# SFXiang/ORB-SLAM2-Annotation

Measured on AMD Instinct MI355X. Metric: frames/sec ORB extract+match (1000 feat, 640×480 mono) at 1/2/4/8 GPU; % HBM roofline, higher is better.
Workload: dtype u8

## Files before the change

### include/orbgpu_debug.h

```cpp
#ifndef ORBGPU_DEBUG_H
#define ORBGPU_DEBUG_H

#include "orbgpu.h"

#ifdef __cplusplus
extern "C" {
#endif

int orbgpu_debug_level_candidates(orbgpu_extractor* ex, int frame, int level, int* xys, int cap);

int orbgpu_debug_level_octree(orbgpu_extractor* ex, int frame, int level, int* xys, int cap);

int orbgpu_debug_level_blur(orbgpu_extractor* ex, int frame, int level, uint8_t* dst, size_t dst_step);

int orbgpu_debug_octree_trace(orbgpu_extractor* ex, int enable, int* out, int cap);

int orbgpu_debug_pyramid_emulate(int nfeatures, float scale_factor, int nlevels, int width, int height,
                                 const uint8_t* img, size_t img_step, uint8_t* out, size_t out_bytes, int* info);

int orbgpu_debug_pyramid_plan_rows(int nfeatures, float scale_factor, int nlevels, int width, int height, int* rows,
                                   size_t rows_n, int* lane_info, size_t lanes_n, int* dims);

int orbgpu_debug_qr_solve_6x4_device(const double* A, const double* b, double* X, int n, void* stream);

#ifdef __cplusplus
}
#endif
#endif
```

### orb-slam2-annotation_amd/csrc/extractor.cpp

```cpp
#include <algorithm>
#include <atomic>
#include <chrono>
#include <cstring>
#include <memory>
#include <string>

#include "extractor.h"

using namespace orbgpu;

namespace {

int pyr_levels_max_batch() { return ORB_ENV_ONCE_INT("ORBGPU_PYR_LEVELS_MAX_BATCH", 8); }

int od_chunks() {
    const int n = env_now_int("ORBGPU_OD_CHUNKS", 1);
    return n < 1 ? 1 : (n > 8 ? 8 : n);
}

bool single_zero_copy() { return ORB_ENV_ONCE_FLAG("ORBGPU_SINGLE_ZEROCOPY", true); }

bool single_done_flag() { return ORB_ENV_ONCE_FLAG("ORBGPU_SINGLE_DONE_FLAG", true); }

bool single_vram_staging() { return ORB_ENV_ONCE_FLAG("ORBGPU_SINGLE_VRAM_STAGING", true); }

bool pyr_bands_off() { return !ORB_ENV_ONCE_FLAG("ORBGPU_PYR_BANDS", true); }

int run_batch(orbgpu_extractor* e, const uint8_t* imgs, int batch, size_t row_step, size_t frame_step,
              orbgpu_keypoint* kps, uint8_t* desc, int* counts, int kp_cap, hipStream_t s, int* err_copy = nullptr) {
    const Geom& g = e->geo.g;
    Event* evs = nullptr;
    if (e->profile) {
        if (e->ev_used == e->ev.size()) {
            std::array<Event, 5> a;
            for (Event& x : a) ORB_HIP(hipEventCreateWithFlags(x.put(), hipEventDisableSystemFence));
            e->ev.push_back(std::move(a));
        }
        evs = e->ev[e->ev_used++].data();
        ORB_HIP(hipEventRecord(evs[0], s));
    }
    if (batch <= pyr_levels_max_batch() && g.bd_nb > 0 && !pyr_bands_off())
        ORB_HIP(launch_pyramid_bands(g, batch, e->d_band, e->d_xtab, e->d_ytab, imgs, row_step, frame_step, e->d_pyr, s));
    else if (batch <= pyr_levels_max_batch())
        ORB_HIP(launch_pyramid_levels(g, batch, e->d_xtab, e->d_ytab, imgs, row_step, frame_step, e->d_pyr, s));
    else
        ORB_HIP(launch_pyramid(g, batch, e->d_pyr_ent, e->d_pyr_tab, imgs, row_step, frame_step, e->d_pyr, s));
    if (evs) ORB_HIP(hipEventRecord(evs[1], s));
    if (e->stage_ev[0]) ORB_HIP(hipEventRecord(e->stage_ev[0], s));
    ORB_HIP(launch_fast_cells(g, batch, imgs, row_step, frame_step, e->d_pyr, e->d_cand, e->d_cell_counts, e->d_err, s));
    if (evs) ORB_HIP(hipEventRecord(evs[2], s));
    if (e->stage_ev[1]) ORB_HIP(hipEventRecord(e->stage_ev[1], s));
    const int nch = (err_copy || batch < 16 * od_chunks()) ? 1 : od_chunks();
    if (nch == 1) {
        ORB_HIP(launch_octree(g, batch, e->d_cand, e->d_cell_counts, e->d_gkeys, e->d_gknode, e->d_oct_out,
                              e->d_oct_count, e->d_err, e->geo.oct_groups, 2, e->d_trace, s));
        if (evs) ORB_HIP(hipEventRecord(evs[3], s));
        if (e->stage_ev[2]) ORB_HIP(hipEventRecord(e->stage_ev[2], s));
        ORB_HIP(launch_describe(g, batch, imgs, row_step, frame_step, e->d_pyr, e->d_oct_out, e->d_oct_count, kps,
                                desc, counts, kp_cap, s, err_copy ? e->d_err.get() : nullptr, err_copy));
    } else {
        if (!e->aux_stream) {
            int lo = 0, hi = 0;
            ORB_HIP(hipDeviceGetStreamPriorityRange(&lo, &hi));
            ORB_HIP(hipStreamCreateWithPriority(e->aux_stream.put(), hipStreamNonBlocking, hi));
            for (Event& x : e->od_ev) ORB_HIP(hipEventCreateWithFlags(x.put(), hipEventDisableTiming));
        }
        hipStream_t a = e->aux_stream;
        for (int c = 0; c < nch; ++c) {
            const int f0 = batch * c / nch, f1 = batch * (c + 1) / nch, nb = f1 - f0;
            ORB_HIP(launch_octree(g, nb, e->d_cand + (size_t)f0 * g.cand_frame,
                                  e->d_cell_counts + (size_t)f0 * g.total_cells,
                                  e->d_gkeys + (size_t)f0 * g.cand_frame, e->d_gknode + (size_t)f0 * g.cand_frame,
                                  e->d_oct_out + (size_t)f0 * g.slots_frame, e->d_oct_count + (size_t)f0 * kOcStride,
                                  e->d_err, e->geo.oct_groups, 2, c == 0 ? e->d_trace.get() : nullptr, s));
            if (c == nch - 1 && evs) ORB_HIP(hipEventRecord(evs[3], s));
            ORB_HIP(hipEventRecord(e->od_ev[c], s));
            ORB_HIP(hipStreamWaitEvent(a, e->od_ev[c], 0));
            ORB_HIP(launch_describe(g, nb, imgs, row_step, frame_step, e->d_pyr, e->d_oct_out, e->d_oct_count, kps,
                                    desc, counts, kp_cap, a, nullptr, nullptr, f0));
        }
        if (e->stage_ev[2]) ORB_HIP(hipEventRecord(e->stage_ev[2], s));
        ORB_HIP(hipEventRecord(e->od_ev[8], a));
        ORB_HIP(hipStreamWaitEvent(s, e->od_ev[8], 0));
    }
    if (evs) ORB_HIP(hipEventRecord(evs[4], s));
    if (e->stage_ev[3]) ORB_HIP(hipEventRecord(e->stage_ev[3], s));
    e->last_img = imgs;
    e->last_row = row_step;
    e->last_frame = frame_step;
    e->last_batch = batch;
    return ORBGPU_OK;
}

std::string capacity_message(int err) {
    std::string m = "kernel capacity overflow:";
    if (err & kErrCellCap) m += " FAST-cell";
    if (err & kErrNodeCap) m += " octree-nodes";
    if (err & kErrKeyCap) m += " octree-keys";
    if (err & kErrSeqCap) m += " octree-seq";
    return m;
}

int collect_errors(orbgpu_extractor* e, hipStream_t s) {
    ORB_HIP(hipStreamSynchronize(s));
    int err = 0;
    ORB_HIP(hipMemcpy(&err, e->d_err, sizeof(int), hipMemcpyDeviceToHost));
    if (err) {
        ORB_HIP(hipMemset(e->d_err, 0, sizeof(int)));
        return fail(ORBGPU_ERR_CAPACITY, capacity_message(err));
    }
    return ORBGPU_OK;
}

template <class T>
hipError_t upload(T* dst, const std::vector<T>& src) {
    return src.empty() ? hipSuccess : hipMemcpy(dst, src.data(), src.size() * sizeof(T), hipMemcpyHostToDevice);
}

}

extern "C" {

int orbgpu_extractor_create(int nfeatures, float scale_factor, int nlevels, int ini_th, int min_th, int width,
                            int height, int max_batch, orbgpu_extractor** out) {
    if (!out) return fail(ORBGPU_ERR_ARG, "out is NULL");
    *out = nullptr;
    if (nfeatures <= 0 || nlevels <= 0 || nlevels > kMaxLevels || !(scale_factor > 1.f) || width <= 0 ||
// ... 352 lines not shown
```

### orb-slam2-annotation_amd/csrc/extractor_debug.cpp

```cpp
#include <algorithm>
#include <cstring>
#include <vector>

#include "../../include/orbgpu_debug.h"
#include "extractor.h"

using namespace orbgpu;

namespace {

int plan_geometry(int nfeatures, float scale_factor, int nlevels, int width, int height, ExtractorGeometry& geo,
                  GeometryTables& t) {
    return build_geometry(ExtractorParams{nfeatures, scale_factor, nlevels, 20, 7, width, height, 1}, geo, t);
}

}

extern "C" {

int orbgpu_debug_level_blur(orbgpu_extractor* e, int frame, int level, uint8_t* dst, size_t dst_step) {
    if (!e || !dst) return fail(ORBGPU_ERR_ARG, "NULL argument");
    DeviceScope ds_(e->device);
    if (!e->last_img || frame < 0 || frame >= e->last_batch || level < 0 || level >= e->p.nlevels)
        return fail(ORBGPU_ERR_ARG, "no such frame/level in the last extraction");
// ... 48 lines not shown
    if (out && e->d_trace) {
        ORB_HIP(hipDeviceSynchronize());
        ORB_HIP(hipMemcpy(out, e->d_trace, std::min(n, (size_t)cap) * sizeof(int), hipMemcpyDeviceToHost));
    }
    return ORBGPU_OK;
}

int orbgpu_debug_level_octree(orbgpu_extractor* e, int frame, int level, int* xys, int cap) {
    if (!e || frame < 0 || frame >= e->last_batch || level < 0 || level >= e->p.nlevels)
        return fail(ORBGPU_ERR_ARG, "no such frame/level in the last extraction");
    DeviceScope ds_(e->device);
    const Geom& g = e->geo.g;
    const LevelGeom& v = g.lv[level];
    int n = 0;
    ORB_HIP(hipDeviceSynchronize());
    ORB_HIP(hipMemcpy(&n, e->d_oct_count + (size_t)frame * kOcStride + level, sizeof(int), hipMemcpyDeviceToHost));
    std::vector<uint32_t> keys(std::max(n, 1));
    ORB_HIP(hipMemcpy(keys.data(), e->d_oct_out + (size_t)frame * g.slots_frame + v.out_offset,
                      (size_t)n * sizeof(uint32_t), hipMemcpyDeviceToHost));
    for (int i = 0; i < n && i < cap && xys; ++i) {
        xys[3 * i] = key_x(keys[i]); xys[3 * i + 1] = key_y(keys[i]); xys[3 * i + 2] = key_s(keys[i]);
    }
    return n;
}

int orbgpu_debug_pyramid_emulate(int nfeatures, float scale_factor, int nlevels, int width, int height,
                                 const uint8_t* img, size_t img_step, uint8_t* out, size_t out_bytes, int* info) {
    if (!img || !out || nfeatures <= 0 || nlevels <= 0 || nlevels > kMaxLevels || !(scale_factor > 1.f) ||
        width <= 0 || height <= 0 || img_step < (size_t)width)
        return fail(ORBGPU_ERR_ARG, "invalid emulation arguments");
    ExtractorGeometry geo;
    GeometryTables t;
    int rc = plan_geometry(nfeatures, scale_factor, nlevels, width, height, geo, t);
    if (rc) return rc;
    const Geom& g = geo.g;
    size_t need = 0;
    for (int l = 1; l < nlevels; ++l) need += (size_t)g.lv[l].w * g.lv[l].h;
    if (out_bytes < need) return fail(ORBGPU_ERR_CAPACITY, "out_bytes smaller than levels 1..L-1");
    std::vector<std::vector<uint8_t>> levels;
    rc = emulate_pyramid(g, t.ytab, geo.pyr_plan, img, img_step, levels);
    if (rc) return rc;
    for (int l = 1; l < nlevels; ++l) {
        std::memcpy(out, levels[(size_t)l].data(), levels[(size_t)l].size());
        out += levels[(size_t)l].size();
    }
    if (info) {
        const int v[8] = {g.tk_ticks, g.tk_t0, g.tk_cwaves, g.tk_pwaves, g.tk_np, g.tk_e, g.tk_lds_bytes,
                          g.lv[0].tk_ring_rows};
        std::memcpy(info, v, sizeof(v));
    }
    return ORBGPU_OK;
}

int orbgpu_debug_pyramid_plan_rows(int nfeatures, float scale_factor, int nlevels, int width, int height,
                                   int* rows, size_t rows_n, int* lane_info, size_t lanes_n, int* dims) {
    if (!dims || nfeatures <= 0 || nlevels < 2 || nlevels > kMaxLevels || !(scale_factor > 1.f) || width <= 0 ||
        height <= 0)
        return fail(ORBGPU_ERR_ARG, "invalid plan arguments");
    ExtractorGeometry geo;
    GeometryTables t;
    int rc = plan_geometry(nfeatures, scale_factor, nlevels, width, height, geo, t);
    if (rc) return rc;
    const Geom& g = geo.g;
    const int K = g.tk_ticks, CL = 64 * g.tk_cwaves, E = g.tk_e, n = CL * E;
    dims[0] = K;
    dims[1] = n;
    dims[2] = g.tk_cwaves;
    dims[3] = E;
    if (!rows || !lane_info) return ORBGPU_OK;
    if (rows_n < (size_t)K * n || lanes_n < (size_t)n) return fail(ORBGPU_ERR_CAPACITY, "plan output too small");
    const uint32_t* rng = reinterpret_cast<const uint32_t*>(geo.pyr_plan.tab.data()) + g.tk_rng;
    for (int i = 0; i < n; ++i) {
        const int4* r = &geo.pyr_plan.ent[(size_t)i * 9];
        lane_info[i] = r[2].w | (r[0].y ? 1 << 8 : 0);
        for (int k = 0; k < K; ++k) rows[(size_t)k * n + i] = (int)((rng[(size_t)k * g.tk_rs + r[0].x] >> 11) & 31u);
    }
    return ORBGPU_OK;
}

}
```

### orb-slam2-annotation_amd/csrc/octree.hip

```cpp
#include "orbgpu_internal.h"
#include "orbgpu_kernels.h"
#include "group_sum.h"
#include <algorithm>
#include <type_traits>

namespace orbgpu {

namespace {

#ifndef ORBGPU_OCT_THREADS
#define ORBGPU_OCT_THREADS 256
#endif
#ifndef ORBGPU_OCT_AGG_HIST
#define ORBGPU_OCT_AGG_HIST 1
#endif
constexpr bool kAggHist = ORBGPU_OCT_AGG_HIST != 0;
constexpr int kThreads = ORBGPU_OCT_THREADS;
#ifndef ORBGPU_OCT_THREADS_SMALL
#define ORBGPU_OCT_THREADS_SMALL 1024
#endif
constexpr int kThreadsSmall = ORBGPU_OCT_THREADS_SMALL;
constexpr int kSmallBatch = 8;

struct ONode {
// ... 169 lines not shown
        const int ex = incl - x;
        const unsigned long long br = __ballot(lane < m && nL + (ex - lane) + x - 1 >= N);
        const int kstop = br ? (int)__builtin_ctzll(br) : m - 1;
        C = kstop >= 0 ? __builtin_amdgcn_readlane(incl, kstop) : 0;
        if (lane == 0) s_misc[24] = kstop;
        if (lane < m) s_aux0[lane] = ex;
        wave_sync();
        flag = div && rank <= kstop;
        base = flag ? s_aux0[rank] : 0;
        const unsigned long long bs = __ballot(valid && !flag);
        S = __popcll(bs);
        spos = lanes_below(bs);
        wave_sync();
    }
    const bool bad = C + S > ncap || nseq + C > 0x0FFFFFFF;
    if (lane == 0) {
        s_misc[20] = C;
        s_misc[21] = S;
        s_misc[22] = bad ? (C + S > ncap ? kErrNodeCap : kErrSeqCap) : 0;
    }
    int nexp = 0;
    if (!bad && valid) {
        s_flag[lane] = flag;
        if (flag) {
            int p = base;
#pragma unroll
            for (int q = 0; q < 4; ++q) {
                const uint32_t c = qc.get(lane, q);
                if (c > 0) {
                    const int pos = C - 1 - p;
                    ONode ch = child_rect(nd, q);
                    ch.cnt = c;
                    ch.seq = (uint32_t)(nseq + p);
                    nw[pos] = ch;
                    qc.set(lane, q, pos);
                    nexp += c > 1;
                    ++p;
                }
            }
        } else {
            const int pos = C + spos;
            nw[pos] = nd;
            s_aux1[lane] = pos;
        }
    }
    const int tot_exp = __popcll(__ballot(nexp >= 1)) + __popcll(__ballot(nexp >= 2)) + __popcll(__ballot(nexp >= 3)) +
                        __popcll(__ballot(nexp >= 4));
    if (lane == 0) *s_nexp = tot_exp;
    const int nNew = C + S;
    if (!bad && (nNew >= N || nNew == nL))
        for (int i = lane; i < nNew; i += 64) s_aux0[i] = 0;
}

template <int NT, bool LDS>
__device__ void octree_body(const Geom& g, const LevelGeom& L, int l, int f, int nk, int ncells, int ncap, int ncap2,
                            const uint32_t* __restrict__ cand, uint32_t* __restrict__ out,
                            int* __restrict__ oct_count, int* __restrict__ err, int* __restrict__ trace,
                            KeyStore<LDS> ks, QuadCounts<LDS> qc, int* s_misc, ONode* s_node0, ONode* s_node1,
                            int* s_aux0, int* s_aux1, uint8_t* s_flag, int* s_cellofs) {
    const int tid = threadIdx.x;
    int* s_tmp = s_misc;

    const int N = L.nfeat;
    const int nini = L.nini;
    if (nini > ncap) {
        if (tid == 0) { atomicOr(err, kErrNodeCap); oct_count[f * kOcStride + l] = 0; }
        return;
    }

    for (int i = tid; i < nini; i += NT) s_aux0[i] = 0;
    OCT_T(60);
    for (int c = tid; c < ncells; c += NT) {
        const int b = s_cellofs[c], e = s_cellofs[c + 1];
        for (int k = b; k < e; ++k) ks.set_node(k, c);
    }
    __syncthreads();
    OCT_T(61);
    const uint32_t* cbase = cand + (size_t)f * g.cand_frame + L.cand_offset;
    const bool one_root = nini == 1;
    constexpr int kGather = 8;
    for (int k0 = tid; k0 < nk; k0 += kGather * NT) {
        uint32_t key[kGather];
#pragma unroll
        for (int u = 0; u < kGather; ++u) {
            const int k = min(k0 + u * NT, nk - 1);
            const int c = ks.node(k);
            key[u] = cbase[(size_t)c * L.cell_cap + (k - s_cellofs[c])];
        }
#pragma unroll
        for (int u = 0; u < kGather; ++u) {
            const int k = k0 + u * NT;
            if (k < nk) {
                ks.set_key(k, key[u]);
                if (one_root) {
                    ks.set_node(k, 0);
                } else {
                    int r = (int)__fdiv_rn((float)key_x(key[u]), L.hx);
                    r = min(r, nini - 1);
                    ks.set_node(k, r);
                    atomicAdd(&s_aux0[r], 1);
                }
            }
        }
    }
    if (one_root && tid == 0) s_aux0[0] = nk;
    __syncthreads();
    OCT_T(1);
    auto make_root = [&](int r, int c, int pos) {
        ONode nd;
        const int x0 = (int)(L.hx * (float)r), x1 = (int)(L.hx * (float)(r + 1));
        nd.r0 = (uint32_t)x0;
        nd.r1 = (uint32_t)x1 | ((uint32_t)(L.max_by - kBorder) << 16);
        nd.cnt = (uint32_t)c;
        nd.seq = (uint32_t)r;
        s_node0[pos] = nd;
    };
    int nroots;
    if (__builtin_amdgcn_readfirstlane(nini) <= 64) {
        if (tid < 64) {
            const int c = tid < nini ? s_aux0[tid] : 0;
            const unsigned long long b = __ballot(c > 0);
            const int pos = lanes_below(b);
            if (c > 0) make_root(tid, c, pos);
            if (tid < nini) s_aux1[tid] = c > 0 ? pos : -1;
            if (tid == 0) s_misc[23] = __popcll(b);
        }
        __syncthreads();
        nroots = s_misc[23];
    } else {
        for (int r = tid; r < nini; r += NT) s_aux1[r] = s_aux0[r] > 0 ? 1 : 0;
        __syncthreads();
        nroots = block_scan<NT>(s_aux1, nini, s_tmp);
        for (int r = tid; r < nini; r += NT) {
            const int c = s_aux0[r];
            const int pos = s_aux1[r];
            if (c > 0) make_root(r, c, pos);
            s_aux1[r] = c > 0 ? pos : -1;
        }
        __syncthreads();
    }
    if (!one_root)
        for (int k = tid; k < nk; k += NT) ks.set_node(k, s_aux1[ks.node(k)]);
    __syncthreads();

    OCT_T(2);
    int nL = nroots, cur = 0, nseq = nini;
    bool inner = false;
    uint32_t* s_best = reinterpret_cast<uint32_t*>(s_aux0);
    int best_state = 0;
    for (int guard = 0; guard < 4096; ++guard) {
        ONode* old = cur ? s_node1 : s_node0;
        ONode* nw = cur ? s_node0 : s_node1;
        unsigned long long* s_sortk = reinterpret_cast<unsigned long long*>(nw);
        int* s_nexp = s_misc + 25 + (guard & 1);
        qc.zero(nL, tid, NT);
        if (tid == 0) *s_nexp = 0;
        __syncthreads();
        if constexpr (kAggHist && NT == kThreads) {
        for (int k0 = tid & ~63; k0 < nk; k0 += NT) {
            const int lane = tid & 63, k = k0 + lane;
            const bool valid = k < nk;
            const int i = valid ? ks.node(k) : -1;
            const int i0 = __builtin_amdgcn_readfirstlane(i);
            const bool uni = __ballot(valid && i != i0) == 0ull;
            const ONode nd = old[valid ? i : i0];
            const int q = valid && nd.cnt > 1 ? node_quad(nd, ks.key(k)) : -1;
            if (uni) {
                const unsigned long long b0 = __ballot(q == 0), b1 = __ballot(q == 1), b2 = __ballot(q == 2),
                                         b3 = __ballot(q == 3);
                if (lane == 0) {
                    if (b0) qc.add(i0, 0, (uint32_t)__popcll(b0));
                    if (b1) qc.add(i0, 1, (uint32_t)__popcll(b1));
                    if (b2) qc.add(i0, 2, (uint32_t)__popcll(b2));
                    if (b3) qc.add(i0, 3, (uint32_t)__popcll(b3));
                }
            } else if (q >= 0) {
                qc.add(i, q);
            }
        }
        } else {
        for (int k = tid; k < nk; k += NT) {
            const int i = ks.node(k);
            const ONode nd = old[i];
            if (nd.cnt > 1) qc.add(i, node_quad(nd, ks.key(k)));
        }
        }
        __syncthreads();
        OCT_T(3 + 4 * guard);
        int C, S;
        const bool small = __builtin_amdgcn_readfirstlane(nL) <= 64;
        if (small) {
            if (tid < 64) wave_small_pass(old, nw, s_sortk, qc, s_aux0, s_aux1, s_flag, s_misc, s_nexp, nL, N, ncap,
                                          nseq, inner, tid);
            __syncthreads();
            C = s_misc[20];
            S = s_misc[21];
            if (s_misc[22]) {
                if (tid == 0) { atomicOr(err, s_misc[22]); oct_count[f * kOcStride + l] = 0; }
                return;
            }
        } else {
            if (!inner) {
                for (int i = tid; i < nL; i += NT) {
// ... 143 lines not shown
            }
            best_state = 2;
        } else {
            for (int k = tid; k < nk; k += NT) {
                const int i = ks.node(k);
                ks.set_node(k, s_flag[i] ? (int)qc.get(i, node_quad(old[i], ks.key(k))) : s_aux1[i]);
            }
            if (done) {
                for (int i = tid; i < nNew; i += NT) s_best[i] = 0;
                best_state = 1;
            }
        }
        __syncthreads();
        OCT_T(6 + 4 * guard);
        if (tid == 0 && trace && f == 0 && guard < 47) {
            int* t = trace + l * 512 + 2 + guard * 8;
            t[0] = inner; t[1] = nL; t[2] = C; t[3] = S; t[4] = *s_nexp; t[5] = s_misc[24]; t[6] = nk; t[7] = N;
            trace[l * 512] = guard + 1;
        }
        const int nexp = *s_nexp;
        if (!inner && nNew + nexp * 3 > N) inner = true;
        nseq += C;
        cur ^= 1;
        nL = nNew;
        if (done) break;
    }

    if (best_state == 0) {
        for (int i = tid; i < nL; i += NT) s_best[i] = 0;
        __syncthreads();
    }
    if (best_state < 2) {
        for (int k = tid; k < nk; k += NT)
            atomicMax(&s_best[ks.node(k)], ((uint32_t)key_s(ks.key(k)) << 24) | (0xFFFFFFu - (uint32_t)k));
        __syncthreads();
    }
    if (nL > L.ocap) {
        if (tid == 0) { atomicOr(err, kErrNodeCap); oct_count[f * kOcStride + l] = 0; }
        return;
    }
    for (int i = tid; i < nL; i += NT) out[i] = ks.key((int)(0xFFFFFFu - (s_best[i] & 0xFFFFFFu)));
    if (tid == 0) oct_count[f * kOcStride + l] = nL;
    OCT_T(63);
}

template <int NT>
__global__ __launch_bounds__(NT) void octree_kernel(Geom g, const uint32_t* __restrict__ cand,
                                                          const int* __restrict__ cell_counts,
                                                          uint32_t* __restrict__ gkeys,
                                                          uint16_t* __restrict__ gknode,
                                                          uint32_t* __restrict__ oct_out,
                                                          int* __restrict__ oct_count, int* __restrict__ err,
                                                          int* __restrict__ trace, OctreeGroup A, OctreeGroup B,
                                                          int batch) {
    extern __shared__ __attribute__((aligned(16))) uint8_t smem[];
    const int id = (int)blockIdx.x, na = A.nlev * batch;
    const bool inA = id < na;
    const OctreeGroup& G = inA ? A : B;
    const int j = inA ? id : id - na;
    const int f = j / G.nlev, l = G.level0 + (j - f * G.nlev);
    const int kcap = G.kcap, ncap = G.ncap;
    const int tid = threadIdx.x;
    const LevelGeom& L = g.lv[l];
    const int ncells = L.ncols * L.nrows;
    const int ncap2 = pow2ceil(ncap);
    OCT_T(0);

    const size_t o_node0 = 128;
    const size_t o_node1 = o_node0 + (size_t)ncap * 16;
    const size_t o_qc = o_node1 + std::max((size_t)ncap * 16, (((size_t)(g.max_cells_level + 1) * 4 + 15) & ~(size_t)15));
    const size_t o_aux0 = o_qc + (size_t)ncap * 8;
    const size_t o_aux1 = o_aux0 + (size_t)ncap * 4;
    const size_t o_flag = o_aux1 + (size_t)ncap * 4;
    const size_t o_keys = o_flag + (size_t)ncap;
    const size_t o_knode = o_keys + (size_t)kcap * 4;
    int* s_misc = reinterpret_cast<int*>(smem);
    ONode* s_node0 = reinterpret_cast<ONode*>(smem + o_node0);
    ONode* s_node1 = reinterpret_cast<ONode*>(smem + o_node1);
    int* s_aux0 = reinterpret_cast<int*>(smem + o_aux0);
    int* s_aux1 = reinterpret_cast<int*>(smem + o_aux1);
    uint8_t* s_flag = smem + o_flag;
    int* s_cellofs = reinterpret_cast<int*>(smem + o_node1);
    int* s_tmp = s_misc;

    const int* cc = cell_counts + (size_t)f * g.total_cells + L.cell_base;
    for (int i = tid; i < ncells; i += NT) s_cellofs[i] = cc[i];
    if (tid == 0) s_cellofs[ncells] = 0;
    __syncthreads();
    const int nk = block_scan<NT>(s_cellofs, ncells + 1, s_tmp);
    uint32_t* out = oct_out + (size_t)f * g.slots_frame + L.out_offset;
    if (nk <= kcap) {
        KeyStore<true> ks{reinterpret_cast<uint32_t*>(smem + o_keys), reinterpret_cast<uint16_t*>(smem + o_knode)};
        QuadCounts<true> qc{reinterpret_cast<uint16_t*>(smem + o_qc)};
        octree_body<NT, true>(g, L, l, f, nk, ncells, ncap, ncap2, cand, out, oct_count, err, trace, ks, qc, s_misc,
                              s_node0, s_node1, s_aux0, s_aux1, s_flag, s_cellofs);
    } else {
        KeyStore<false> ks{gkeys + (size_t)f * g.cand_frame + L.cand_offset,
                           gknode + (size_t)f * g.cand_frame + L.cand_offset};
        QuadCounts<false> qc{reinterpret_cast<uint32_t*>(smem + o_keys)};
        octree_body<NT, false>(g, L, l, f, nk, ncells, ncap, ncap2, cand, out, oct_count, err, trace, ks, qc, s_misc,
                               s_node0, s_node1, s_aux0, s_aux1, s_flag, s_cellofs);
    }
}

}

size_t octree_lds_bytes(const Geom& g, int kcap, int ncap) {
    auto r16 = [](size_t b) { return (b + 15) & ~(size_t)15; };
    const size_t n = (size_t)ncap;
    return r16(32 * 4) + r16(n * 16) + std::max(r16(n * 16), r16((size_t)(g.max_cells_level + 1) * 4)) +
           r16(n * 8) + 2 * r16(n * 4) + r16(n) +
           std::max(r16((size_t)kcap * 4) + r16((size_t)kcap * 2), r16(n * 16));
}

hipError_t launch_octree(const Geom& g, int batch, const uint32_t* cand, const int* cell_counts,
                         uint32_t* gkeys, uint16_t* gknode, uint32_t* oct_out, int* oct_count,
                         int* err, const OctreeGroup* groups, int ngroups, int* trace, hipStream_t stream) {
    const bool small = batch <= kSmallBatch;
    auto kernel = small ? &octree_kernel<kThreadsSmall> : &octree_kernel<kThreads>;
    const int nt = small ? kThreadsSmall : kThreads;
    if (ngroups == 2 && groups[0].nlev > 0 && groups[1].nlev > 0) {
        const size_t lds = std::max(octree_lds_bytes(g, groups[0].kcap, groups[0].ncap),
                                    octree_lds_bytes(g, groups[1].kcap, groups[1].ncap));
        hipLaunchKernelGGL(kernel, dim3((groups[0].nlev + groups[1].nlev) * batch), dim3(nt), lds,
                           stream, g, cand, cell_counts, gkeys, gknode, oct_out, oct_count, err, trace, groups[0],
                           groups[1], batch);
        return hipGetLastError();
    }
    for (int i = 0; i < ngroups; ++i) {
        const OctreeGroup& G = groups[i];
        if (G.nlev <= 0) continue;
        const size_t lds = octree_lds_bytes(g, G.kcap, G.ncap);
        hipLaunchKernelGGL(kernel, dim3(G.nlev * batch), dim3(nt), lds, stream, g, cand, cell_counts,
                           gkeys, gknode, oct_out, oct_count, err, trace, G, OctreeGroup{0, 0, 0, 0}, batch);
        const hipError_t e = hipGetLastError();
        if (e != hipSuccess) return e;
    }
    return hipSuccess;
}

}
```

### orb-slam2-annotation_amd/csrc/orbgpu_kernels.h

```cpp
#pragma once

#include <vector>

#include "orbgpu_internal.h"

struct orbgpu_keypoint;
struct orbgpu_pack_desc;

namespace orbgpu {

struct PyrPlan {
    std::vector<int2> tab;
    std::vector<int4> ent;
};
int plan_pyramid(Geom& g, const std::vector<int2>& ytab, const std::vector<int4>& ptab, int max_batch, PyrPlan& plan);
int slot_offset(const Geom& g, int l, int r);
int emulate_pyramid(const Geom& g, const std::vector<int2>& ytab, const PyrPlan& plan, const uint8_t* img, size_t row0,
                    std::vector<std::vector<uint8_t>>& levels);
hipError_t launch_pyramid_levels(const Geom& g, int batch, const int2* xtab, const int2* ytab, const uint8_t* img0,
                                 size_t row0, size_t frame0, uint8_t* pyr, hipStream_t stream);
void plan_pyramid_bands(Geom& g, const std::vector<int2>& ytab, std::vector<int4>& bands);
hipError_t launch_pyramid_bands(const Geom& g, int batch, const int4* bands, const int2* xtab, const int2* ytab,
                                const uint8_t* img0, size_t row0, size_t frame0, uint8_t* pyr, hipStream_t stream);
hipError_t launch_pyramid(const Geom& g, int batch, const int4* ents, const int2* tab, const uint8_t* img0,
                          size_t row0, size_t frame0, uint8_t* pyr, hipStream_t stream);
hipError_t pyramid_set_lds_limit(const Geom& g);

hipError_t launch_fast_cells(const Geom& g, int batch, const uint8_t* img0, size_t row0, size_t frame0,
                             const uint8_t* pyr, uint32_t* cand, int* cell_counts, int* err,
                             hipStream_t stream);

hipError_t launch_blur_levels(const Geom& g, int batch, const uint8_t* img0, size_t row0, size_t frame0,
                              const uint8_t* pyr, uint8_t* blur, hipStream_t stream, int level_from = 0);

size_t octree_lds_bytes(const Geom& g, int kcap, int ncap);
struct OctreeGroup {
    int level0, nlev, kcap, ncap;
};
hipError_t launch_octree(const Geom& g, int batch, const uint32_t* cand, const int* cell_counts,
                         uint32_t* gkeys, uint16_t* gknode, uint32_t* oct_out, int* oct_count,
                         int* err, const OctreeGroup* groups, int ngroups, int* trace, hipStream_t stream);

hipError_t launch_describe(const Geom& g, int batch, const uint8_t* img0, size_t row0, size_t frame0,
                           const uint8_t* pyr, const uint32_t* oct_out, const int* oct_count,
                           orbgpu_keypoint* kps, uint8_t* desc, int* counts, int kp_cap,
                           hipStream_t stream, int* err_word = nullptr, int* err_copy = nullptr, int f0 = 0);

struct MatchFirstF1 {
    const orbgpu_keypoint* kps = nullptr;
    const uint8_t* desc = nullptr;
    const int* n = nullptr;
};

hipError_t launch_match_init(int batch, float minX, float maxX, float minY, float maxY,
                             const orbgpu_keypoint* kps1, const uint8_t* desc1, const int* n1, size_t stride1,
                             const orbgpu_keypoint* kps2, const uint8_t* desc2, const int* n2, size_t stride2,
                             float* prev_xy, int window, float nnratio, int flags,
                             int* matches12, int* nmatches, hipStream_t stream, size_t level0_bound = 0,
                             MatchFirstF1 first = MatchFirstF1());

hipError_t launch_hamming_pairs(const uint8_t* a, const uint8_t* b, int n, int* dist, hipStream_t stream);
hipError_t launch_pack_rows(int batch, int cap, int ntensors, const ::orbgpu_pack_desc* d, hipStream_t stream);
hipError_t launch_copy16(void* dst, const void* src, size_t nbytes, hipStream_t stream);
hipError_t launch_done_flag(unsigned long long* flag, unsigned long long v, hipStream_t stream);
constexpr int kCopyList = 16;
struct CopyDesc16 {
    const void* src;
    void* dst;
    size_t bytes;
};
struct CopyList16 {
    CopyDesc16 d[kCopyList];
    int n;
};
hipError_t launch_copy16_list(const CopyList16& L, hipStream_t stream);

enum : int {
    kErrCellCap = 1,
    kErrNodeCap = 2,
    kErrKeyCap = 4,
    kErrUnused8 = 8,
    kErrSeqCap = 16,
};

}
```

### orb-slam2-annotation_amd/orbgpu.py

```python
from __future__ import annotations

import ctypes
import os
from pathlib import Path

import numpy as np

_HERE = Path(__file__).resolve().parent
LIB_PATH = Path(os.environ.get("ORBGPU_LIBRARY", str(_HERE / "liborbgpu.so")))
_LIB = None

OK, ERR_ARG, ERR_HIP, ERR_CAPACITY, ERR_UNSUPPORTED, ERR_NO_DEVICE = 0, -1, -2, -3, -4, -5
MATCH_CHECK_ORI = 1
MATCH_ANNOTATED_HISTO = 2
COLOR_RGB, COLOR_BGR, COLOR_RGBA, COLOR_BGRA = 0, 1, 2, 3
DEPTH_U16, DEPTH_F32 = 0, 1

KP_DTYPE = np.dtype([("x", "<f4"), ("y", "<f4"), ("size", "<f4"), ("angle", "<f4"),
                     ("response", "<f4"), ("octave", "<i4"), ("class_id", "<i4")])


class OrbGpuError(RuntimeError):
    def __init__(self, code: int, what: str):
        super().__init__(f"{what} failed ({code}): {last_error()}")
# ... 33 lines not shown
class _Info(ctypes.Structure):
    _fields_ = [("nlevels", ctypes.c_int), ("width", ctypes.c_int), ("height", ctypes.c_int),
                ("max_batch", ctypes.c_int), ("max_keypoints", ctypes.c_int),
                ("level_width", ctypes.c_int * 32), ("level_height", ctypes.c_int * 32),
                ("features_per_level", ctypes.c_int * 32), ("level_capacity", ctypes.c_int * 32),
                ("device", ctypes.c_int)]


def lib() -> ctypes.CDLL:
    global _LIB
    if _LIB is None:
        if not LIB_PATH.exists():
            raise RuntimeError(f"HIP extension not built: {LIB_PATH} (run __graft_entry__.build())")
        try:
            import torch
        except ImportError:
            pass
        L = ctypes.CDLL(str(LIB_PATH))
        vp, i, f, sz = ctypes.c_void_p, ctypes.c_int, ctypes.c_float, ctypes.c_size_t
        L.orbgpu_last_error.restype = ctypes.c_char_p
        L.orbgpu_device_arch.argtypes = [ctypes.c_char_p, i]
        L.orbgpu_extractor_create.argtypes = [i, f, i, i, i, i, i, i, ctypes.POINTER(vp)]
        L.orbgpu_extractor_create_on_device.argtypes = [i, i, f, i, i, i, i, i, i, ctypes.POINTER(vp)]
        L.orbgpu_extractor_destroy.argtypes = [vp]
        L.orbgpu_device_event_create.argtypes = [ctypes.POINTER(vp)]
        L.orbgpu_device_event_destroy.argtypes = [vp]
        L.orbgpu_device_event_record.argtypes = [vp, vp]
        L.orbgpu_stream_wait_device_event.argtypes = [vp, vp]
        L.orbgpu_device_count.argtypes = [ctypes.POINTER(i)]
        L.orbgpu_set_thread_device.argtypes = [i]
        L.orbgpu_get_thread_device.argtypes = [ctypes.POINTER(i)]
        L.orbgpu_extractor_get_info.argtypes = [vp, ctypes.POINTER(_Info)]
        L.orbgpu_extractor_get_scales.argtypes = [vp, vp, vp, vp, vp]
        L.orbgpu_extract.argtypes = [vp, vp, i, i, sz, vp, vp, i, ctypes.POINTER(i)]
        L.orbgpu_extract_batch_device.argtypes = [vp, vp, i, sz, sz, vp, vp, vp, i, vp]
        L.orbgpu_extractor_sync.argtypes = [vp, vp]
        L.orbgpu_extractor_profile.argtypes = [vp, i]
        L.orbgpu_extractor_stage_times.argtypes = [vp, vp, ctypes.POINTER(i), i]
        L.orbgpu_extractor_set_stage_event.argtypes = [vp, i, vp]
        L.orbgpu_extractor_copy_level.argtypes = [vp, i, i, vp, sz]
        L.orbgpu_hamming_pairs_device.argtypes = [vp, vp, i, vp, vp]
        L.orbgpu_pack_rows_device.argtypes = [i, i, i, ctypes.POINTER(PackDesc), vp]
        L.orbgpu_search_for_initialization_batch_device.argtypes = [
            i, GridBounds, vp, vp, vp, sz, vp, vp, vp, sz, vp, i, f, i, vp, vp, vp]
        L.orbgpu_search_for_initialization_batch_device_bounded.argtypes = [
            i, GridBounds, vp, vp, vp, sz, vp, vp, vp, sz, vp, i, f, i, i, vp, vp, vp]
        L.orbgpu_search_for_initialization_stream_device.argtypes = [
            i, GridBounds, vp, vp, vp, sz, vp, vp, vp, vp, i, f, i, i, vp, vp, vp]
        L.orbgpu_debug_level_candidates.argtypes = [vp, i, i, vp, i]
        L.orbgpu_debug_level_blur.argtypes = [vp, i, i, vp, sz]
        L.orbgpu_debug_level_octree.argtypes = [vp, i, i, vp, i]
        L.orbgpu_debug_octree_trace.argtypes = [vp, i, vp, i]
        L.orbgpu_debug_pyramid_emulate.argtypes = [i, f, i, i, i, vp, sz, vp, sz, vp]
        L.orbgpu_search_for_initialization.argtypes = [GridBounds, vp, vp, i, vp, vp, i, vp, i, f, i, vp,
                                                       ctypes.POINTER(i)]
        L.orbgpu_compute_image_bounds.argtypes = [ctypes.POINTER(Camera), i, i, ctypes.POINTER(GridBounds)]
        L.orbgpu_undistort_keypoints_batch_device.argtypes = [ctypes.POINTER(Camera), i, vp, vp, i, vp, vp]
        L.orbgpu_assign_features_to_grid_batch_device.argtypes = [i, GridBounds, vp, vp, i, vp, vp, vp]
        L.orbgpu_stereo_matches_batch_device.argtypes = [vp, vp, sz, sz, i, vp, vp, vp, i, f, f, vp, vp, vp]
        L.orbgpu_gray_from_color_batch_device.argtypes = [vp, i, i, i, i, sz, sz, vp, sz, sz, vp]
        L.orbgpu_stereo_from_rgbd_batch_device.argtypes = [vp, i, f, i, i, sz, sz, i, vp, vp, vp, i,
                                                           ctypes.POINTER(Camera), f, vp, vp, vp, vp]
        L.orbgpu_pose_optimization_batch_device.argtypes = [i, vp, i, vp, vp, vp, vp, vp, vp]
        L.orbgpu_pose_optimization_batch.argtypes = [i, vp, i, vp, vp, vp, vp, vp]
        L.orbgpu_optimize_sim3_batch_device.argtypes = [i, vp, i, vp, vp, vp, vp, vp, vp, vp, vp, vp]
        L.orbgpu_optimize_sim3_batch.argtypes = [i, vp, i, vp, vp, vp, vp, vp, vp, vp, vp]
        L.orbgpu_local_ba_workspace_bytes.argtypes = [i, i, i, i, i]
        L.orbgpu_local_ba_workspace_bytes.restype = sz
        L.orbgpu_local_ba_batch_device.argtypes = [i, vp, i, i, i, i, i] + [vp] * 13 + [sz, vp]
        L.orbgpu_local_ba_batch.argtypes = [i, vp, i, i, i, i, i] + [vp] * 13 + [sz]
        L.orbgpu_srand.argtypes = [ctypes.c_uint]
        L.orbgpu_srand.restype = None
        L.orbgpu_rand.restype = i
        L.orbgpu_random_int.argtypes = [i, i]
        L.orbgpu_rand_get_state.argtypes = [vp]
        L.orbgpu_rand_get_state.restype = None
        L.orbgpu_rand_set_state.argtypes = [vp]
        L.orbgpu_rand_set_state.restype = None
        L.orbgpu_srand_r.argtypes = [vp, ctypes.c_uint]
        L.orbgpu_srand_r.restype = None
        L.orbgpu_rand_r.argtypes = [vp]
        L.orbgpu_sim3_workspace_bytes.argtypes = [i]
        L.orbgpu_sim3_workspace_bytes.restype = sz
        L.orbgpu_sim3_ransac_batch_device.argtypes = [i, vp, i, vp, vp, vp, vp, vp, vp, vp, vp, vp]
        L.orbgpu_sim3_ransac_batch.argtypes = [i, vp, i, vp, vp, vp, vp, i, vp, vp, vp]
        L.orbgpu_pnp_workspace_bytes.argtypes = [i, i]
        L.orbgpu_pnp_workspace_bytes.restype = sz
        L.orbgpu_pnp_ransac_batch_device.argtypes = [i, vp, i, i, i, vp, vp, vp, vp, vp, vp, vp, vp, vp]
        L.orbgpu_pnp_ransac_batch.argtypes = [i, vp, i, vp, vp, vp, i, vp, vp, vp, vp]
        L.orbgpu_vocabulary_load_text.argtypes = [ctypes.c_char_p, ctypes.POINTER(vp)]
        L.orbgpu_vocabulary_load_binary.argtypes = [ctypes.c_char_p, ctypes.POINTER(vp)]
        L.orbgpu_vocabulary_create.argtypes = [i, i, i, i, i, vp, vp, vp, vp, ctypes.POINTER(vp)]
        L.orbgpu_vocabulary_destroy.argtypes = [vp]
        L.orbgpu_vocabulary_get_info.argtypes = [vp, vp]
        L.orbgpu_bow_transform_batch_device.argtypes = [vp, i, vp, vp, i, i, vp, vp, vp, vp, vp, vp, vp, vp, vp, vp,
                                                        vp]
        L.orbgpu_bow_transform.argtypes = [vp, i, vp, i, vp, vp, vp, vp, vp, vp, vp, vp, vp, vp]
        L.orbgpu_search_by_bow_batch_device.argtypes = [i, i, vp, vp, f, i, i, vp, vp, vp]
        L.orbgpu_search_by_bow.argtypes = [i, vp, vp, f, i, vp, vp]
        L.orbgpu_is_in_frustum_device.argtypes = [vp, i, vp, vp, vp, vp, f, vp, vp, vp, vp]
        L.orbgpu_search_by_projection_batch_device.argtypes = [i, vp, i, vp, vp, vp]
        L.orbgpu_search_by_projection.argtypes = [vp, vp, vp]
        L.orbgpu_search_by_sim3.argtypes = [vp, vp, vp]
        _LIB = L
    return _LIB

# ... 1 lines not shown
def last_error() -> str:
    return lib().orbgpu_last_error().decode(errors="replace")


def _check(rc: int, what: str) -> None:
    if rc != OK:
        raise OrbGpuError(rc, what)


def device_arch() -> str:
    buf = ctypes.create_string_buffer(64)
    _check(lib().orbgpu_device_arch(buf, 64), "orbgpu_device_arch")
    return buf.value.decode()


def device_count() -> int:
    n = ctypes.c_int()
    _check(lib().orbgpu_device_count(ctypes.byref(n)), "orbgpu_device_count")
    return n.value


def set_thread_device(device: int) -> None:
    _check(lib().orbgpu_set_thread_device(int(device)), "orbgpu_set_thread_device")


def get_thread_device() -> int:
    d = ctypes.c_int()
    _check(lib().orbgpu_get_thread_device(ctypes.byref(d)), "orbgpu_get_thread_device")
    return d.value


def pyramid_plan_emulate(img: np.ndarray, nfeatures=1000, scale_factor=1.2, nlevels=8):
    img = np.ascontiguousarray(img, dtype=np.uint8)
    h, w = img.shape
    sizes, s = [], np.float32(1.0)
    for l in range(1, nlevels):
        s = np.float32(s * np.float32(scale_factor))
        inv = np.float32(np.float32(1.0) / s)
        sizes.append((int(np.rint(np.float32(h) * inv)), int(np.rint(np.float32(w) * inv))))
    out = np.zeros(sum(a * b for a, b in sizes) + 64, np.uint8)
    info = np.zeros(8, np.int32)
    _check(lib().orbgpu_debug_pyramid_emulate(nfeatures, scale_factor, nlevels, w, h, img.ctypes.data, img.strides[0],
                                              out.ctypes.data, out.size, info.ctypes.data),
           "orbgpu_debug_pyramid_emulate")
    levels, o = [], 0
    for lh, lw in sizes:
        levels.append(out[o:o + lw * lh].reshape(lh, lw).copy())
        o += lw * lh
    keys = ("ticks", "rows_per_chunk", "compute_waves", "producer_waves", "loads_per_lane", "entries_per_lane",
            "lds_bytes", "ring0_rows")
    return levels, dict(zip(keys, (int(v) for v in info)))


def _ptr(a) -> int:
    if hasattr(a, "data_ptr"):
        return a.data_ptr()
    return a.ctypes.data


def _stream_ptr(stream) -> int | None:
    if stream is None:
        return None
    return getattr(stream, "cuda_stream", stream)


class DeviceEvent:

    def __init__(self):
        h = ctypes.c_void_p()
        _check(lib().orbgpu_device_event_create(ctypes.byref(h)), "device_event_create")
        self.cuda_event = h.value
        self._lib = lib()

    @staticmethod
    def _stream(stream):
        if stream is None:
            import torch
            stream = torch.cuda.current_stream()
        return stream.cuda_stream

    def record(self, stream=None):
        _check(lib().orbgpu_device_event_record(self.cuda_event, self._stream(stream)), "device_event_record")

    def wait(self, stream=None):
        _check(lib().orbgpu_stream_wait_device_event(self._stream(stream), self.cuda_event), "stream_wait_device_event")

    def __del__(self):
        try:
            if self.cuda_event:
                self._lib.orbgpu_device_event_destroy(self.cuda_event)
        except Exception:
            pass


class Extractor:

    def __init__(self, nfeatures=1000, scale_factor=1.2, nlevels=8, ini_th=20, min_th=7,
                 width=640, height=480, max_batch=1, device=None):
        h = ctypes.c_void_p()
        if device is None:
            _check(lib().orbgpu_extractor_create(nfeatures, scale_factor, nlevels, ini_th, min_th,
                                                 width, height, max_batch, ctypes.byref(h)),
                   "orbgpu_extractor_create")
        else:
            _check(lib().orbgpu_extractor_create_on_device(int(device), nfeatures, scale_factor, nlevels, ini_th,
                                                           min_th, width, height, max_batch, ctypes.byref(h)),
# ... 251 lines not shown
```

Measured before the change: 465,300.

## Fuse first three octree subdivision passes into one key sweep plus wave replay

Adds a fused octree path, on by default, for levels with at most four roots. A single sweep over the keys computes each key's depth-3 quadrant bin and builds a histogram in LDS. One wave then replays up to three subdivision passes from the aggregated counts, and keys are remapped to their nodes through a lookup table. This replaces several per-pass full sweeps and barriers over all keys. In exchange it can raise LDS usage through the kFusedBytes floor and adds complexity.

```diff
diff --git a/include/orbgpu_debug.h b/include/orbgpu_debug.h
--- a/include/orbgpu_debug.h
+++ b/include/orbgpu_debug.h
@@ -18,6 +18,8 @@
 int orbgpu_debug_pyramid_emulate(int nfeatures, float scale_factor, int nlevels, int width, int height,
                                  const uint8_t* img, size_t img_step, uint8_t* out, size_t out_bytes, int* info);
 
+int orbgpu_debug_octree_plan(int nfeatures, float scale_factor, int nlevels, int width, int height, int* out);
+
 int orbgpu_debug_pyramid_plan_rows(int nfeatures, float scale_factor, int nlevels, int width, int height, int* rows,
                                    size_t rows_n, int* lane_info, size_t lanes_n, int* dims);
 
diff --git a/orb-slam2-annotation_amd/csrc/extractor.cpp b/orb-slam2-annotation_amd/csrc/extractor.cpp
--- a/orb-slam2-annotation_amd/csrc/extractor.cpp
+++ b/orb-slam2-annotation_amd/csrc/extractor.cpp
@@ -23,6 +23,8 @@
 bool single_done_flag() { return ORB_ENV_ONCE_FLAG("ORBGPU_SINGLE_DONE_FLAG", true); }
 
 bool single_vram_staging() { return ORB_ENV_ONCE_FLAG("ORBGPU_SINGLE_VRAM_STAGING", true); }
+
+bool oct_fused() { return env_now_int("ORBGPU_OCT_FUSED", 1) != 0; }
 
 bool pyr_bands_off() { return !ORB_ENV_ONCE_FLAG("ORBGPU_PYR_BANDS", true); }
 
@@ -53,7 +55,7 @@
     const int nch = (err_copy || batch < 16 * od_chunks()) ? 1 : od_chunks();
     if (nch == 1) {
         ORB_HIP(launch_octree(g, batch, e->d_cand, e->d_cell_counts, e->d_gkeys, e->d_gknode, e->d_oct_out,
-                              e->d_oct_count, e->d_err, e->geo.oct_groups, 2, e->d_trace, s));
+                              e->d_oct_count, e->d_err, e->geo.oct_groups, 2, e->d_trace, oct_fused(), s));
         if (evs) ORB_HIP(hipEventRecord(evs[3], s));
         if (e->stage_ev[2]) ORB_HIP(hipEventRecord(e->stage_ev[2], s));
         ORB_HIP(launch_describe(g, batch, imgs, row_step, frame_step, e->d_pyr, e->d_oct_out, e->d_oct_count, kps,
@@ -72,7 +74,7 @@
                                   e->d_cell_counts + (size_t)f0 * g.total_cells,
                                   e->d_gkeys + (size_t)f0 * g.cand_frame, e->d_gknode + (size_t)f0 * g.cand_frame,
                                   e->d_oct_out + (size_t)f0 * g.slots_frame, e->d_oct_count + (size_t)f0 * kOcStride,
-                                  e->d_err, e->geo.oct_groups, 2, c == 0 ? e->d_trace.get() : nullptr, s));
+                                  e->d_err, e->geo.oct_groups, 2, c == 0 ? e->d_trace.get() : nullptr, oct_fused(), s));
             if (c == nch - 1 && evs) ORB_HIP(hipEventRecord(evs[3], s));
             ORB_HIP(hipEventRecord(e->od_ev[c], s));
             ORB_HIP(hipStreamWaitEvent(a, e->od_ev[c], 0));
diff --git a/orb-slam2-annotation_amd/csrc/extractor_debug.cpp b/orb-slam2-annotation_amd/csrc/extractor_debug.cpp
--- a/orb-slam2-annotation_amd/csrc/extractor_debug.cpp
+++ b/orb-slam2-annotation_amd/csrc/extractor_debug.cpp
@@ -124,6 +124,22 @@
     return ORBGPU_OK;
 }
 
+int orbgpu_debug_octree_plan(int nfeatures, float scale_factor, int nlevels, int width, int height, int* out) {
+    if (!out || nfeatures <= 0 || nlevels <= 0 || nlevels > kMaxLevels || !(scale_factor > 1.f) || width <= 0 ||
+        height <= 0)
+        return fail(ORBGPU_ERR_ARG, "invalid octree plan arguments");
+    ExtractorGeometry geo;
+    GeometryTables t;
+    const int rc = plan_geometry(nfeatures, scale_factor, nlevels, width, height, geo, t);
+    if (rc) return rc;
+    for (int i = 0; i < 2; ++i) {
+        const OctreeGroup& G = geo.oct_groups[i];
+        const int v[5] = {G.level0, G.nlev, G.kcap, G.ncap, (int)octree_lds_bytes(geo.g, G.kcap, G.ncap)};
+        std::memcpy(out + 5 * i, v, sizeof(v));
+    }
+    return ORBGPU_OK;
+}
+
 int orbgpu_debug_pyramid_plan_rows(int nfeatures, float scale_factor, int nlevels, int width, int height,
                                    int* rows, size_t rows_n, int* lane_info, size_t lanes_n, int* dims) {
     if (!dims || nfeatures <= 0 || nlevels < 2 || nlevels > kMaxLevels || !(scale_factor > 1.f) || width <= 0 ||
diff --git a/orb-slam2-annotation_amd/csrc/octree.hip b/orb-slam2-annotation_amd/csrc/octree.hip
--- a/orb-slam2-annotation_amd/csrc/octree.hip
+++ b/orb-slam2-annotation_amd/csrc/octree.hip
@@ -245,12 +245,145 @@
         for (int i = lane; i < nNew; i += 64) s_aux0[i] = 0;
 }
 
+constexpr int kFusedRoots = 4;
+constexpr int kFusedTabOfs = kFusedRoots * 84 * 4;
+constexpr int kFusedTagOfs = kFusedTabOfs + kFusedRoots * 64 * 2;
+constexpr int kFusedBytes = kFusedTagOfs + 2 * 256 * 2;
+static_assert(kFusedBytes % 16 == 0, "the key region behind the fused scratch stays 16-byte aligned");
+
+template <int NT, class KS>
+__device__ void fused_sweep(const KS& ks, const ONode* roots, int* s_bins, int nk) {
+    const int tid = threadIdx.x, lane = tid & 63;
+    for (int k0 = tid & ~63; k0 < nk; k0 += NT) {
+        const int k = k0 + lane;
+        const bool valid = k < nk;
+        int bin = -1;
+        if (valid) {
+            const int r = ks.node(k);
+            const uint32_t key = ks.key(k);
+            ONode nd = roots[r];
+            const int q1 = node_quad(nd, key);
+            nd = child_rect(nd, q1);
+            const int q2 = node_quad(nd, key);
+            nd = child_rect(nd, q2);
+            const int q3 = node_quad(nd, key);
+            bin = (r << 6) | (q1 << 4) | (q2 << 2) | q3;
+            ks.set_node(k, bin);
+        }
+        const int prev = __shfl_up(bin, 1);
+        const bool head = lane == 0 || bin != prev;
+        const unsigned long long rest = (__ballot(head) >> lane) >> 1;
+        const int len = rest ? (int)__builtin_ctzll(rest) + 1 : 64 - lane;
+        if (head && valid) atomicAdd(&s_bins[bin], len);
+    }
+}
+
+__device__ inline void wave_replay(ONode* s_node0, ONode* s_node1, uint8_t* s_fused, int* s_misc, int nroots, int nini,
+                                   int N, int ncap, int nk, int l, int f, int* trace, int lane) {
+    int* s_bins = reinterpret_cast<int*>(s_fused);
+    uint16_t* s_tab = reinterpret_cast<uint16_t*>(s_fused + kFusedTabOfs);
+    uint16_t* s_tag = reinterpret_cast<uint16_t*>(s_fused + kFusedTagOfs);
+    int* A3 = s_bins;
+    int* A2 = s_bins + nroots * 64;
+    int* A1 = s_bins + nroots * 80;
+    for (int j = lane; j < nroots * 16; j += 64) {
+        const int4 v = reinterpret_cast<const int4*>(A3)[j];
+        A2[j] = v.x + v.y + v.z + v.w;
+    }
+    wave_sync();
+    if (lane < nroots * 4) {
+        const int4 v = reinterpret_cast<const int4*>(A2)[lane];
+        A1[lane] = v.x + v.y + v.z + v.w;
+    }
+    if (lane < nroots) s_tag[lane] = (uint16_t)lane;
+    wave_sync();
+    int nL = nroots, cur = 0, nseq = nini, npass = 0;
+    bool inner = false;
+    for (int p = 1; p <= 3; ++p) {
+        if (nL > 64) break;
+        const ONode* old = cur ? s_node1 : s_node0;
+        ONode* nw = cur ? s_node0 : s_node1;
+        const uint16_t* tag_old = s_tag + cur * 256;
+        uint16_t* tag_nw = s_tag + (cur ^ 1) * 256;
+        const bool valid = lane < nL;
+        ONode nd{};
+        int tag = 0;
+        if (valid) {
+            nd = old[lane];
+            tag = tag_old[lane];
+        }
+        const bool div = valid && nd.cnt > 1;
+        const int gid = tag & 0xFFF;
+        int4 c = make_int4(0, 0, 0, 0);
+        if (div) c = reinterpret_cast<const int4*>(p == 1 ? A1 : (p == 2 ? A2 : A3))[gid];
+        const int nch = (c.x != 0) + (c.y != 0) + (c.z != 0) + (c.w != 0);
+        const int nexp = (c.x > 1) + (c.y > 1) + (c.z > 1) + (c.w > 1);
+        const int v = valid ? (div ? nch << 16 : 1) : 0;
+        const int incl = wave_incl_scan_dpp(v);
+        const int tot = __builtin_amdgcn_readlane(incl, 63);
+        const int C = tot >> 16, S = tot & 0xFFFF, nNew = C + S;
+        const bool bad = nNew > ncap || nseq + C > 0x0FFFFFFF;
+        const bool done = nNew >= N || nNew == nL;
+        if (bad || done) break;
+        const int tot_exp = __popcll(__ballot(nexp >= 1)) + __popcll(__ballot(nexp >= 2)) +
+                            __popcll(__ballot(nexp >= 3)) + __popcll(__ballot(nexp >= 4));
+        if (div) {
+            int pp = (incl - v) >> 16;
+            const int cq[4] = {c.x, c.y, c.z, c.w};
+#pragma unroll
+            for (int q = 0; q < 4; ++q)
+                if (cq[q] > 0) {
+                    const int pos = C - 1 - pp;
+                    ONode ch = child_rect(nd, q);
+                    ch.cnt = (uint32_t)cq[q];
+                    ch.seq = (uint32_t)(nseq + pp);
+                    nw[pos] = ch;
+                    tag_nw[pos] = (uint16_t)((gid * 4 + q) | (p << 12));
+                    ++pp;
+                }
+        } else if (valid) {
+            const int pos = C + ((incl - v) & 0xFFFF);
+            nw[pos] = nd;
+            tag_nw[pos] = (uint16_t)tag;
+        }
+        if (lane == 0 && trace && f == 0) {
+            int* t = trace + l * 512 + 2 + (p - 1) * 8;
+            t[0] = 0; t[1] = nL; t[2] = C; t[3] = S; t[4] = tot_exp; t[5] = -1; t[6] = nk; t[7] = N;
+            trace[l * 512] = p;
+        }
+        wave_sync();
+        nseq += C;
+        cur ^= 1;
+        nL = nNew;
+        npass = p;
+        if (nNew + tot_exp * 3 > N) {
+            inner = true;
+            break;
+        }
+    }
+    const uint16_t* tag_cur = s_tag + cur * 256;
+    for (int i = lane; i < nL; i += 64) {
+        const int tag = tag_cur[i];
+        const int sh = 2 * (3 - (tag >> 12));
+        const int b0 = (tag & 0xFFF) << sh;
+        for (int j = 0; j < (1 << sh); ++j) s_tab[b0 + j] = (uint16_t)i;
+    }
+    if (lane == 0) {
+        s_misc[27] = nL;
+        s_misc[28] = cur;
+        s_misc[29] = nseq;
+        s_misc[30] = inner;
+        s_misc[31] = npass;
+        if (trace && f == 0) trace[l * 512 + 1] = 1 + npass;
+    }
+}
+
 template <int NT, bool LDS>
 __device__ void octree_body(const Geom& g, const LevelGeom& L, int l, int f, int nk, int ncells, int ncap, int ncap2,
                             const uint32_t* __restrict__ cand, uint32_t* __restrict__ out,
                             int* __restrict__ oct_count, int* __restrict__ err, int* __restrict__ trace,
                             KeyStore<LDS> ks, QuadCounts<LDS> qc, int* s_misc, ONode* s_node0, ONode* s_node1,
-                            int* s_aux0, int* s_aux1, uint8_t* s_flag, int* s_cellofs) {
+                            int* s_aux0, int* s_aux1, uint8_t* s_flag, int* s_cellofs, uint8_t* s_fused, bool fused) {
     const int tid = threadIdx.x;
     int* s_tmp = s_misc;
 
@@ -337,11 +470,34 @@
     __syncthreads();
 
     OCT_T(2);
-    int nL = nroots, cur = 0, nseq = nini;
+    int nL = nroots, cur = 0, nseq = nini, guard0 = 0;
     bool inner = false;
+    const int nroots_u = __builtin_amdgcn_readfirstlane(nroots);
+    if (fused && nroots_u >= 1 && nroots_u <= kFusedRoots) {
+        int* s_bins = reinterpret_cast<int*>(s_fused);
+        const uint16_t* s_tab = reinterpret_cast<const uint16_t*>(s_fused + kFusedTabOfs);
+        for (int i = tid; i < nroots * 84; i += NT) s_bins[i] = 0;
+        __syncthreads();
+        fused_sweep<NT>(ks, s_node0, s_bins, nk);
+        __syncthreads();
+        OCT_T(56);
+        if (tid < 64) wave_replay(s_node0, s_node1, s_fused, s_misc, nroots, nini, N, ncap, nk, l, f, trace, tid);
+        __syncthreads();
+        OCT_T(57);
+        nL = s_misc[27];
+        cur = s_misc[28];
+        nseq = s_misc[29];
+        inner = s_misc[30] != 0;
+        guard0 = s_misc[31];
+        for (int k = tid; k < nk; k += NT) ks.set_node(k, (int)s_tab[ks.node(k)]);
+        __syncthreads();
+        OCT_T(58);
+    } else if (tid == 0 && trace && f == 0) {
+        trace[l * 512 + 1] = 0;
+    }
     uint32_t* s_best = reinterpret_cast<uint32_t*>(s_aux0);
     int best_state = 0;
-    for (int guard = 0; guard < 4096; ++guard) {
+    for (int guard = guard0; guard < 4096; ++guard) {
         ONode* old = cur ? s_node1 : s_node0;
         ONode* nw = cur ? s_node0 : s_node1;
         unsigned long long* s_sortk = reinterpret_cast<unsigned long long*>(nw);
@@ -591,7 +747,7 @@
                                                           uint32_t* __restrict__ oct_out,
                                                           int* __restrict__ oct_count, int* __restrict__ err,
                                                           int* __restrict__ trace, OctreeGroup A, OctreeGroup B,
-                                                          int batch) {
+                                                          int batch, int fused) {
     extern __shared__ __attribute__((aligned(16))) uint8_t smem[];
     const int id = (int)blockIdx.x, na = A.nlev * batch;
     const bool inA = id < na;
@@ -611,7 +767,7 @@
     const size_t o_aux0 = o_qc + (size_t)ncap * 8;
     const size_t o_aux1 = o_aux0 + (size_t)ncap * 4;
     const size_t o_flag = o_aux1 + (size_t)ncap * 4;
-    const size_t o_keys = o_flag + (size_t)ncap;
+    const size_t o_keys = o_qc + std::max((size_t)ncap * 17, (size_t)kFusedBytes);
     const size_t o_knode = o_keys + (size_t)kcap * 4;
     int* s_misc = reinterpret_cast<int*>(smem);
     ONode* s_node0 = reinterpret_cast<ONode*>(smem + o_node0);
@@ -632,13 +788,13 @@
         KeyStore<true> ks{reinterpret_cast<uint32_t*>(smem + o_keys), reinterpret_cast<uint16_t*>(smem + o_knode)};
         QuadCounts<true> qc{reinterpret_cast<uint16_t*>(smem + o_qc)};
         octree_body<NT, true>(g, L, l, f, nk, ncells, ncap, ncap2, cand, out, oct_count, err, trace, ks, qc, s_misc,
-                              s_node0, s_node1, s_aux0, s_aux1, s_flag, s_cellofs);
+                              s_node0, s_node1, s_aux0, s_aux1, s_flag, s_cellofs, smem + o_qc, fused != 0);
     } else {
         KeyStore<false> ks{gkeys + (size_t)f * g.cand_frame + L.cand_offset,
                            gknode + (size_t)f * g.cand_frame + L.cand_offset};
         QuadCounts<false> qc{reinterpret_cast<uint32_t*>(smem + o_keys)};
         octree_body<NT, false>(g, L, l, f, nk, ncells, ncap, ncap2, cand, out, oct_count, err, trace, ks, qc, s_misc,
-                               s_node0, s_node1, s_aux0, s_aux1, s_flag, s_cellofs);
+                               s_node0, s_node1, s_aux0, s_aux1, s_flag, s_cellofs, smem + o_qc, fused != 0);
     }
 }
 
@@ -648,13 +804,13 @@
     auto r16 = [](size_t b) { return (b + 15) & ~(size_t)15; };
     const size_t n = (size_t)ncap;
     return r16(32 * 4) + r16(n * 16) + std::max(r16(n * 16), r16((size_t)(g.max_cells_level + 1) * 4)) +
-           r16(n * 8) + 2 * r16(n * 4) + r16(n) +
+           std::max(r16(n * 8) + 2 * r16(n * 4) + r16(n), (size_t)kFusedBytes) +
            std::max(r16((size_t)kcap * 4) + r16((size_t)kcap * 2), r16(n * 16));
 }
 
 hipError_t launch_octree(const Geom& g, int batch, const uint32_t* cand, const int* cell_counts,
                          uint32_t* gkeys, uint16_t* gknode, uint32_t* oct_out, int* oct_count,
-                         int* err, const OctreeGroup* groups, int ngroups, int* trace, hipStream_t stream) {
+                         int* err, const OctreeGroup* groups, int ngroups, int* trace, bool fused, hipStream_t stream) {
     const bool small = batch <= kSmallBatch;
     auto kernel = small ? &octree_kernel<kThreadsSmall> : &octree_kernel<kThreads>;
     const int nt = small ? kThreadsSmall : kThreads;
@@ -663,7 +819,7 @@
                                     octree_lds_bytes(g, groups[1].kcap, groups[1].ncap));
         hipLaunchKernelGGL(kernel, dim3((groups[0].nlev + groups[1].nlev) * batch), dim3(nt), lds,
                            stream, g, cand, cell_counts, gkeys, gknode, oct_out, oct_count, err, trace, groups[0],
-                           groups[1], batch);
+                           groups[1], batch, fused ? 1 : 0);
         return hipGetLastError();
     }
     for (int i = 0; i < ngroups; ++i) {
@@ -671,7 +827,7 @@
         if (G.nlev <= 0) continue;
         const size_t lds = octree_lds_bytes(g, G.kcap, G.ncap);
         hipLaunchKernelGGL(kernel, dim3(G.nlev * batch), dim3(nt), lds, stream, g, cand, cell_counts,
-                           gkeys, gknode, oct_out, oct_count, err, trace, G, OctreeGroup{0, 0, 0, 0}, batch);
+                           gkeys, gknode, oct_out, oct_count, err, trace, G, OctreeGroup{0, 0, 0, 0}, batch, fused ? 1 : 0);
         const hipError_t e = hipGetLastError();
         if (e != hipSuccess) return e;
     }
diff --git a/orb-slam2-annotation_amd/csrc/orbgpu_kernels.h b/orb-slam2-annotation_amd/csrc/orbgpu_kernels.h
--- a/orb-slam2-annotation_amd/csrc/orbgpu_kernels.h
+++ b/orb-slam2-annotation_amd/csrc/orbgpu_kernels.h
@@ -39,7 +39,7 @@
 };
 hipError_t launch_octree(const Geom& g, int batch, const uint32_t* cand, const int* cell_counts,
                          uint32_t* gkeys, uint16_t* gknode, uint32_t* oct_out, int* oct_count,
-                         int* err, const OctreeGroup* groups, int ngroups, int* trace, hipStream_t stream);
+                         int* err, const OctreeGroup* groups, int ngroups, int* trace, bool fused, hipStream_t stream);
 
 hipError_t launch_describe(const Geom& g, int batch, const uint8_t* img0, size_t row0, size_t frame0,
                            const uint8_t* pyr, const uint32_t* oct_out, const int* oct_count,
diff --git a/orb-slam2-annotation_amd/orbgpu.py b/orb-slam2-annotation_amd/orbgpu.py
--- a/orb-slam2-annotation_amd/orbgpu.py
+++ b/orb-slam2-annotation_amd/orbgpu.py
@@ -109,6 +109,7 @@
         L.orbgpu_debug_level_octree.argtypes = [vp, i, i, vp, i]
         L.orbgpu_debug_octree_trace.argtypes = [vp, i, vp, i]
         L.orbgpu_debug_pyramid_emulate.argtypes = [i, f, i, i, i, vp, sz, vp, sz, vp]
+        L.orbgpu_debug_octree_plan.argtypes = [i, f, i, i, i, vp]
         L.orbgpu_search_for_initialization.argtypes = [GridBounds, vp, vp, i, vp, vp, i, vp, i, f, i, vp,
                                                        ctypes.POINTER(i)]
         L.orbgpu_compute_image_bounds.argtypes = [ctypes.POINTER(Camera), i, i, ctypes.POINTER(GridBounds)]
@@ -216,6 +217,14 @@
     return levels, dict(zip(keys, (int(v) for v in info)))
 
 
+def octree_plan(nfeatures=1000, scale_factor=1.2, nlevels=8, width=640, height=480):
+    out = np.zeros(10, np.int32)
+    _check(lib().orbgpu_debug_octree_plan(nfeatures, scale_factor, nlevels, width, height, out.ctypes.data),
+           "orbgpu_debug_octree_plan")
+    keys = ("level0", "levels", "kcap", "ncap", "lds_bytes")
+    return [dict(zip(keys, (int(v) for v in out[5 * g:5 * g + 5]))) for g in range(2)]
+
+
 def _ptr(a) -> int:
     if hasattr(a, "data_ptr"):
         return a.data_ptr()
```

Result: faster. 474,900 (median of 6 runs) (+2.1%).
